# luchsonice/3dod

Measured on AMD Instinct MI355X. Metric: images/sec Cube R-CNN DLA34-FPN train step, higher is better.
Workload: dtype fp32; 1 GPU; Cube R-CNN DLA34+FPN train step (fwd+loss+bwd+allreduce+SGD), 4 img/GPU 512x512, Base_Omni3D.yaml semantics (BASELINE configs[3] per-GPU shard); global_batch=4, parallelism=dp1, weight_gradient_reduce=pixel splits stored and added in a fixed order (CR_DETERMINISTIC=1), valid=True

## Files before the change

3dod_amd/_lib.py:

```python
import ctypes
import os
import threading

import torch

_HERE = os.path.dirname(os.path.abspath(__file__))
LIB_PATH = os.path.join(_HERE, "lib", "libcr3dod.so")

c_void_p, c_int, c_int64, c_float = ctypes.c_void_p, ctypes.c_int, ctypes.c_int64, ctypes.c_float
P = c_void_p

SIGNATURES = {
    "cr_ctx_create": [c_int, P, ctypes.POINTER(P)],
    "cr_ctx_destroy": [P],
    "cr_ctx_set_stream": [P, P],
    "cr_abi_version": [],
    "cr_cuboid_corners": [P, P, P, c_int64, P],
    "cr_cubes_project_score": [P, P, c_int64, c_int64, P, c_int, c_float, c_float, P, P, P, P,
                               P, P, P, P, P, P, P, P, P],
    "cr_cubes_project_score_fast": [P, P, c_int64, c_int64, P, c_int, c_float, c_float, P, P, P, P,
                                    P, P, P, P, P, P, P, P, P, P],
    "cr_propose": [P, P, c_int64, P, c_int, c_int, P, P, P, c_int64, P, c_int, P, P, P, P, P],
    "cr_ransac_plane": [P, P, c_int64, P, c_int64, c_float, P, P, P],
    "cr_ransac_plane_batched": [P, P, P, c_int, c_int64, P, c_int64, c_float, P, P, P],
# ... 18 lines not shown
    "cr_rpn_unpack": [P, P, P, c_int, c_int, c_int, c_int, P, P, P],
    "cr_rpn_pack_grad": [P, P, P, P, P, c_int, c_int, c_int, c_int],
    "cr_topk_blocks": [c_int64, c_int],
    "cr_topk": [P, P, c_int, c_int64, c_int, P, P, P],
    "cr_multi_seg": [P, P, c_int, c_int64, c_int],
    "cr_loss_guard": [P, P, c_int, c_float, P, P, P, c_int, c_float, c_float, P],
    "cr_step_counters": [P, P, P, P],
    "cr_weights_split3": [P, P, P, P, c_int, c_int64],
    "cr_conv2d_bwd_weight": [P, P, P, P, c_int, c_int, c_int, c_int, c_int, c_int, c_int, c_int, c_int, c_int],
    "cr_conv2d_bwd_weight_bias": [P, P, P, P, P, c_int, c_int, c_int, c_int, c_int, c_int, c_int, c_int, c_int, c_int],
    "cr_cast_f32_to_bf16": [P, P, P, c_int64],
    "cr_weight_transpose": [P, P, P, c_int, c_int, c_int, c_int],
    "cr_colsum_accum": [P, P, c_int, c_int64, c_int, P, P],
    "cr_bn_fwd": [P, P, P, c_int, P, P, P, P, c_int64, c_int, c_int, c_float, c_float, P, P, P, c_int],
    "cr_bn_bwd": [P, P, P, P, P, P, P, P, P, P, P, c_int64, c_int, c_int, c_int],
    "cr_bn_frozen_unfold": [P, P, P, P, P, P, P, c_float, P, c_int, P, P, c_int, c_int],
    "cr_pool2x_fwd": [P, P, P, c_int, c_int, c_int, c_int, c_int, c_int],
    "cr_pool2x_bwd": [P, P, P, P, c_int, c_int, c_int, c_int, c_int, c_int, P],
    "cr_upsample2x_add": [P, P, P, P, c_int, c_int, c_int, c_int, c_int],
    "cr_sum2x2": [P, P, P, c_int, c_int, c_int, c_int, c_int],
    "cr_preprocess": [P, P, P, c_int, c_int, c_int, P, P, c_int],
    "cr_roi_align_fwd": [P, P, P, P, P, c_int, c_int, P, c_int64, c_int, c_int, P, c_int],
    "cr_roi_align_bwd": [P, P, P, P, P, c_int, c_int, P, c_int64, c_int, c_int, P, c_int],
    "cr_conv2d_fwd_group": [P, c_int, P, P, P, P, P, P, c_int, c_int, c_int, c_int, P, P, c_int, c_int],
    "cr_wino_filter": [P, P, P, c_int, c_int, c_int],
    "cr_gemm_batched_f32": [P, P, P, P, c_int, c_int, c_int, c_int, c_int64, c_int64, c_int64],
    "cr_wino_input": [P, c_int, P, P, P, P, c_int, P, c_int64],
    "cr_wino_output": [P, c_int, P, P, P, P, P, c_int, c_int64, P, c_int, P],
    "cr_wino_dy": [P, c_int, P, P, P, P, c_int, P, c_int64, P],
    "cr_wino_filter_grad": [P, P, P, c_int, c_int, P, P],
    "cr_wgrad_batched_f32": [P, P, P, P, c_int, c_int, c_int, c_int, c_int64, c_int64, c_int64],
    "cr_conv2d_bwd_data_group": [P, c_int, P, P, P, P, P, P, c_int, c_int, c_int, c_int, c_int, P],
    "cr_conv2d_bwd_weight_group": [P, c_int, P, P, P, P, P, P, P, c_int, c_int, c_int, c_int, c_int],
    "cr_roi_align_bwd_set": [P, P, P, P, P, c_int, c_int, c_int, P, c_int64, c_int, c_int, P, c_int],
    "cr_nms_grouped": [P, P, P, c_int, c_int, c_float, P, P],
    "cr_cube_loss_fwd": [P, P, c_int64, c_int, c_int, c_int, c_int, P, P],
    "cr_cube_loss_bwd": [P, P, c_int64, c_int, c_int, c_int, c_int, P, P, P, P, P, P],
    "cr_rpn_decode_select": [P, P, P, P, P, c_int, c_int, c_int, P, c_float, P, c_float, P, P, P],
    "cr_box_match": [P, P, c_int, P, P, c_int, c_int, c_int, P, P, P, P],
    "cr_rpn_label": [P, P, P, P, P, P, P, c_int, c_int, c_int, c_float, c_float, P, c_float, P, P, P, P],
    "cr_rpn_scatter": [P, P, P, c_int, P, P, c_int, c_int, P, c_float, c_int, c_int, P],
    "cr_rpn_loss": [P, P, P, P, P, P, P, c_int, c_int, c_int, P, P, P, P, P],
    "cr_roi_label": [P, P, P, P, P, P, P, c_int, c_int, c_int, c_int, c_float, c_float, c_float, P, P, P],
    "cr_roi_compact": [P, P, P, c_int, P, P, c_int, c_int, P, P, P, c_int, c_int, P, P, P, P, P],
    "cr_box_loss": [P, P, P, P, P, P, P, P, c_int, c_int, c_int, c_int, P, c_float, P, P, P, P, P],
    "cr_det_scores": [P, P, c_int, P, c_int, P, P, c_int, c_int, c_int, c_int, c_float, P, P],
    "cr_det_gather": [P, P, P, P, c_int, P, P, c_int, c_int, c_int, c_int, c_int, P, c_float, P, P, P, P],
    "cr_nms_grouped_cls": [P, P, P, P, c_int, c_int, c_float, P, P],
    "cr_det_pick": [P, P, P, P, P, P, P, P, P, c_int, c_int, c_int, c_int, c_int, c_int, P, P, P, P, P, P],
    "cr_weak_loss_fwd": [P, P, P, P, P, P, P, P, P, c_int, c_int, c_int, c_int, c_int, c_int, P, P, P, P, P],
    "cr_weak_loss_reduce": [P, P, P, P, P, c_int, c_int, P, P, P, c_int, c_int, c_int, c_int, c_int, c_int, P, P, P, P, P, P, P, P,
                            P, P, P],
    "cr_weak_loss_bwd": [P, P, P, P, P, P, P, P, P, c_int, c_int, c_int, c_int, c_int, c_int, P, P, P, P, P, P, P, P, P, P, P, P],
    "cr_cube_select": [P, P, c_int, P, c_int, P, P, P, c_int, c_int, c_int, c_int, P, P, P, P, P, P, P, c_int, c_int, P, P, P],
    "cr_cube_select_bwd": [P, P, c_int, P, c_int, c_int, c_int, P, P, P, P, P, P, P, P, P, c_int, c_int, P, P, P],
    "cr_cube_reduce": [P, P, P, P, P, c_int, c_int, P, P, P],
    "cr_cube_reduce_bwd": [P, P, P, P, c_int, c_int, P, P, P, P],
    "cr_cube_select_norm": [P, P, c_int, P, c_int, c_int, c_int, P, c_int, c_int, P, P, P, P],
    "cr_cube_nondis_fwd": [P, P, P, c_int64, c_int, c_int, c_int, c_int, P, P],
    "cr_cube_nondis_bwd": [P, P, P, c_int64, c_int, c_int, c_int, c_int, P, P, P, P, P, P, P],
    "cr_cube_select_bwd_zraw": [P, c_int, P, c_int, c_int, c_int, P, P, P, P, c_int, P, P],
    "cr_weights_prepare": [P, P, P, P, P, P, c_int, c_int],
    "cr_fc_weight_prepare": [P, P, P, c_int, c_int, c_int, c_int],
    "cr_fc_grad_accum": [P, P, P, c_int, c_int, c_int, c_int],
    "cr_linear_fwd": [P, P, P, P, P, c_int, c_int, c_int, c_int, c_int, c_int, P],
    "cr_linear_bwd_data": [P, P, P, P, c_int, c_int, c_int, c_int, P],
# ... 104 lines not shown
```

3dod_amd/csrc/conv.hip:

```cpp
#include "cr_common.h"
#include "cr_elem.h"
#include <stdlib.h>
#include <type_traits>

typedef __bf16 bf16x8 __attribute__((ext_vector_type(8)));
typedef __bf16 bf16x4 __attribute__((ext_vector_type(4)));
typedef short s16x4 __attribute__((ext_vector_type(4)));
typedef float f32x4 __attribute__((ext_vector_type(4)));

#define CONV_T 256

struct ConvP {
    const void* x;
    const void* w;
    void* y;
    const void* res;
    const float* bias;
    float* stats;
    int N, Hin, Win, Cin, Hout, Wout, Cout;
    int stride, pad, Kdim, M, cshift, relu;
    unsigned x_bytes, w_bytes;
    int f32;
    float* part;
    int ksplit, kstages;
// ... 1717 lines not shown
            for (int j = 0; j < TJ; ++j) {
                const int kk = q0 + noff + j * 16 + li;
#pragma unroll
                for (int e = 0; e < 4; ++e) {
                    const int ch = c0 + moff + i * 16 + 4 * g + e;
                    if (kk < p.Kdim && ch < p.Cout) atomicAdd(&p.dw[(size_t)ch * p.Kdim + kk], acc[i][j][e]);
                }
            }
    } else {
        float* tile = reinterpret_cast<float*>(smem);
#pragma unroll
        for (int gg = 0; gg < KG; ++gg) {
            if (grp == gg) {
#pragma unroll
                for (int i = 0; i < TI; ++i)
#pragma unroll
                    for (int j = 0; j < TJ; ++j)
#pragma unroll
                        for (int e = 0; e < 4; ++e) {
                            float* d = &tile[(moff + i * 16 + 4 * g + e) * TNP + noff + j * 16 + li];
                            if (gg == 0) *d = acc[i][j][e]; else *d += acc[i][j][e];
                        }
            }
            __syncthreads();
        }
        for (int idx = threadIdx.x; idx < TM * TN; idx += CONV_T * KG) {
            const int chl = idx / TN, kl = idx - chl * TN;
            const int ch = c0 + chl, kk = q0 + kl;
            if (kk < p.Kdim && ch < p.Cout) atomicAdd(&p.dw[(size_t)ch * p.Kdim + kk], tile[chl * TNP + kl]);
        }
    }
}

template <int TM, int KS>
__device__ __forceinline__ void conv_wgrad_f32_body(const WgP& p, const int blk_id, const int blk_count) {
    constexpr int TN = 128, KU = 2, PS = 16;
    constexpr int WM = (TM == 128) ? 2 : 1, WN = 4 / WM;
    constexpr int WTM = TM / WM, WTN = TN / WN;
    constexpr int TI = WTM / 16, TJ = WTN / 16;
    constexpr int PP = ((TM + 16) % 32 == 16) ? TM + 16 : TM + 32, PQ = TN + 16;
    constexpr int CPR = TM / 4;
    constexpr int NP = (PS * CPR + CONV_T - 1) / CONV_T;
    __shared__ __attribute__((aligned(16))) float smem[KU * PS * (PP + PQ)];
    float* sP = smem;
    float* sQ = smem + KU * PS * PP;
    const float* __restrict__ xg = reinterpret_cast<const float*>(p.x);
    (void)xg;

    const int tid = threadIdx.x, lane = tid & 63, wave = tid >> 6;
    const int bid = xcd_swizzle(blk_id, blk_count);
    const int bx = bid % p.tm, by = (bid / p.tm) % p.tn, bz = bid / (p.tm * p.tn);
    const int c0 = bx * TM, q0 = by * TN;
    const int step0 = bz * p.steps_per_split;
    const int nsteps_total = (p.M + PS - 1) / PS;
    const int step1 = min(step0 + p.steps_per_split, nsteps_total);
    if (step0 >= step1) return;

    const int qc = tid & 31;
    const int qk = q0 + qc * 4;
    int qr = 0, qs = 0, qch = qk;
    const bool qvalid = qk < p.Kdim;
    if (KS > 1) {
        const int tap = qk >> p.cshift;
        qch = qk & (p.Cin - 1);
        qr = tap / KS;
        qs = tap - qr * KS;
    }
    int pn[2], pho[2], pwo[2];
    {
        const int hw = p.Hout * p.Wout;
#pragma unroll
        for (int i = 0; i < 2; ++i) {
            const int m = step0 * PS + (tid >> 5) + 8 * i;
            pn[i] = m / hw;
            const int rem = m - pn[i] * hw;
            pho[i] = rem / p.Wout;
// ... 241 lines not shown
    for (int j = 0; j < NCH; ++j) {
        const int f = ((j + (int)blockIdx.x) % NCH) * 256 + tid;
        if (f < NW) {
            const int co = f / (TAPS * CIN), k = f - co * (TAPS * CIN);
            const int i = (k >> 4) * 256 + co * 16 + (k & 15);
            const float v = (sRed[i] + sRed[NT * 256 + i]) + (sRed[2 * NT * 256 + i] + sRed[3 * NT * 256 + i]);
            if (p.slab) p.slab[(size_t)blockIdx.x * p.slab_stride + f] = v;
            else atomicAdd(&p.dw[f], v);
        }
    }
    if (p.dbias != nullptr) {
#pragma unroll
        for (int off = 16; off < 64; off <<= 1) bsum += __shfl_xor(bsum, off, 64);
        if (lane < 16) atomicAdd(&p.dbias[lane], bsum);
    }
}

static int try_launch_wgrad_patch_f32(cr_ctx* ctx, WgP& p, int ks) {
    const bool shape_ok = p.Cout == 16 && p.stride == 1 && p.pad == ks / 2 && (p.Hout & 15) == 0 && (p.Wout & 15) == 0 &&
                          p.Hin == p.Hout && p.Win == p.Wout && ((ks == 3 && p.Cin == 16) || (ks == 7 && p.Cin == 4));
    if (!shape_ok) return NOT_TAKEN;
    const int tiles_x = p.Wout / 16, tiles_per_img = tiles_x * (p.Hout / 16), tiles_total = tiles_per_img * p.N;
    const dim3 grid((unsigned)std::min(tiles_total, 256 * PATCH_BLOCKS_PER_CU));
    size_t ws_off = 0;
    if (deterministic_on() && p.dbias) return NOT_TAKEN;
    const bool slabs = wgrad_use_slabs(ctx, p, (int)grid.x, &ws_off);
    if (ks == 3) hipLaunchKernelGGL((k_conv_wgrad_patch_f32<3, 16>), grid, dim3(256), 0, ctx->stream, p, tiles_x, tiles_per_img, tiles_total);
    else hipLaunchKernelGGL((k_conv_wgrad_patch_f32<7, 4>), grid, dim3(256), 0, ctx->stream, p, tiles_x, tiles_per_img, tiles_total);
    if (slabs) wgrad_reduce_slabs(ctx, p, (int)grid.x);
    CR_LAUNCH_CHECK();
    return CR_OK;
}

template <int KS>
static int launch_wgrad_f32_ks(cr_ctx* ctx, WgP& p) {
    constexpr int PS = 16;
    const int nsteps = (p.M + PS - 1) / PS;
    const int tn = (int)cr_cdiv(p.Kdim, 128);
    int TM = p.Cout >= 128 ? 128 : (p.Cout >= 64 ? 64 : (p.Cout >= 32 ? 32 : 16));
    if (TM == 128 && ((p.Cout == 128 && p.M <= 16384) || (p.Cout == 256 && p.M <= 4096))) TM = 64;
    if (TM == 128 && KS == 1 && p.Cout >= 1024) TM = 64;
    const int tm = (int)cr_cdiv(p.Cout, TM);
    const int tiles = tm * tn;
    const int max_splits = nsteps / 8 > 1 ? nsteps / 8 : 1;
    int splits = 768 / tiles;
    if (tiles > 768 && nsteps >= 32) splits = 2;
    if (splits > max_splits) splits = max_splits;
    if (splits > nsteps) splits = nsteps;
    if (splits < 1) splits = 1;
    p.steps_per_split = (nsteps + splits - 1) / splits;
    p.steps_per_split = (p.steps_per_split + 1) & ~1;
    splits = (nsteps + p.steps_per_split - 1) / p.steps_per_split;
    dim3 grid(tm * tn * splits);
    p.tm = tm; p.tn = tn;
    size_t ws_off = 0;
    const bool slabs = wgrad_use_slabs(ctx, p, splits, &ws_off);
    if (TM == 128) hipLaunchKernelGGL((k_conv_wgrad_f32<128, KS>), grid, dim3(CONV_T), 0, ctx->stream, p);
    else if (TM == 64) hipLaunchKernelGGL((k_conv_wgrad_f32<64, KS>), grid, dim3(CONV_T), 0, ctx->stream, p);
    else if (TM == 32) hipLaunchKernelGGL((k_conv_wgrad_f32<32, KS>), grid, dim3(CONV_T), 0, ctx->stream, p);
    else hipLaunchKernelGGL((k_conv_wgrad_f32<16, KS>), grid, dim3(CONV_T), 0, ctx->stream, p);
    if (slabs) wgrad_reduce_slabs(ctx, p, splits);
    CR_LAUNCH_CHECK();
    return CR_OK;
}

template <int TM, int KS>
__global__ __launch_bounds__(CONV_T * 2) void k_conv_wgrad_s3(WgP p) {
    constexpr int TN = 128;
    constexpr int WM = (TM == 128) ? 2 : 1, WN = 4 / WM;
    constexpr int WTM = TM / WM, WTN = TN / WN;
    constexpr int TI = WTM / 16, TJ = WTN / 16;
    constexpr int PP = TM == 128 ? 144 : TM + 8, PQ = TN + 16;
    auto rotQ = [](int row, int col) { return (col + (((row >> 3) & 1) << 6)) & 127; };
    auto rotP = [&](int row, int col) { return TM == 128 ? rotQ(row, col) : col; };
    constexpr int CPR = TM / 8;
    constexpr int NP = (32 * CPR + CONV_T - 1) / CONV_T;
    constexpr int PE = 32 * PP, QE = 32 * PQ;
    constexpr int GE = 3 * (PE + QE);
    constexpr int TNP = TN + 4;
    static_assert(TM * TNP * 4 <= 2 * GE * 2, "reduction tile must fit in the operand images");
    __shared__ __attribute__((aligned(16))) u16 smem[2 * GE];
    const int grp = (int)(threadIdx.x >> 8);
    u16* sP = smem + grp * GE;
    u16* sQ = sP + 3 * PE;

    const int tid = threadIdx.x & (CONV_T - 1), lane = tid & 63, wave = tid >> 6;
    const int bid = xcd_swizzle(blockIdx.x, gridDim.x);
// ... 558 lines not shown
    const int tm = Cout / 128, tn = (int)cr_cdiv((int64_t)ks * ks * Cin, 128), tiles = tm * tn;
    int splits_all = 768 / tiles > 1 ? 768 / tiles : 1;
    int sps = (int)cr_cdiv(steps_all, splits_all);
    if (sps < 8) sps = 8;
    sps = (sps + 1) & ~1;
    for (int i = 0; i < n; ++i) {
        CR_CHECK_ARG(dys[i] && xs[i] && dws[i], "cr_conv2d_bwd_weight_group: NULL tensor %d", i);
        int rc = conv_common_checks("cr_conv2d_bwd_weight_group", Ns[i], Hs[i], Ws[i], Cin, Cout, ks, 1, pad, act_f32);
        if (rc) return rc;
        const int H = Hs[i], W = Ws[i], Ho = H + 2 * pad - ks + 1, Wo = W + 2 * pad - ks + 1;
        WgP& p = g.p[i];
        p = make_wgrad_params(dys[i], xs[i], dws[i], Ns[i], H, W, Cin, Ho, Wo, Cout, ks, 1, pad, act_f32);
        p.dbias = dbiases ? dbiases[i] : nullptr;
        const int nsteps = (p.M + PS - 1) / PS;
        p.steps_per_split = sps;
        p.tm = tm; p.tn = tn;
        counts[i] = tiles * (int)cr_cdiv(nsteps, sps);
    }
    size_t ws_off = 0;
    bool slabs = deterministic_on();
    for (int i = 0; i < n && slabs; ++i) slabs = wgrad_use_slabs(ctx, g.p[i], counts[i] / tiles, &ws_off);
    if (!slabs)
        for (int i = 0; i < n; ++i) { g.p[i].slab = nullptr; g.p[i].bslab = nullptr; g.p[i].slab_stride = 0; }
    const int total = group_starts(n, counts, g.start);
    for (int i = 0; i < n; ++i) g.count[i] = counts[i];
    for (int i = n; i < CR_MAX_GROUP; ++i) { g.start[i] = total; g.count[i] = 0; }
    const dim3 grid((unsigned)total), block(CONV_T);
    if (ks == 1) hipLaunchKernelGGL(k_conv_wgrad_f32_grp<1>, grid, block, 0, ctx->stream, g);
    else hipLaunchKernelGGL(k_conv_wgrad_f32_grp<3>, grid, block, 0, ctx->stream, g);
    if (slabs)
        for (int i = 0; i < n; ++i) wgrad_reduce_slabs(ctx, g.p[i], counts[i] / tiles);
    CR_LAUNCH_CHECK();
    return CR_OK;
}

__global__ void k_cast_f32_bf16(const float* __restrict__ src, u16* __restrict__ dst, int64_t n) {
    const int64_t i = ((int64_t)blockIdx.x * blockDim.x + threadIdx.x) * 4;
    if (i + 3 < n) {
        const float4 v = *reinterpret_cast<const float4*>(src + i);
        uint2 pk;
        pk.x = (unsigned)f2bf(v.x) | ((unsigned)f2bf(v.y) << 16);
        pk.y = (unsigned)f2bf(v.z) | ((unsigned)f2bf(v.w) << 16);
        *reinterpret_cast<uint2*>(dst + i) = pk;
    } else {
        for (int64_t j = i; j < n; ++j) dst[j] = f2bf(src[j]);
    }
}

template <typename T>
__global__ __launch_bounds__(256) void k_fold_bn(const float* __restrict__ w, const float* __restrict__ gamma,
                                                 const float* __restrict__ beta, const float* __restrict__ mean,
                                                 const float* __restrict__ var, float eps, T* __restrict__ wf,
                                                 float* __restrict__ bias, int Cout, int K) {
    const int co = blockIdx.x;
    const float s = gamma[co] * rsqrtf(var[co] + eps);
    if (threadIdx.x == 0) bias[co] = beta[co] - mean[co] * s;
    const float* wr = w + (size_t)co * K;
    T* o = wf + (size_t)co * K;
    for (int i = threadIdx.x; i < K; i += 256) {
        if constexpr (sizeof(T) == 2) o[i] = f2bf(wr[i] * s); else o[i] = wr[i] * s;
    }
}

extern "C" int cr_fold_bn(cr_ctx* ctx, const float* w, const float* gamma, const float* beta, const float* mean,
                          const float* var, float eps, void* wf, float* bias, int Cout, int K, int act_f32) {
    CR_CHECK_ARG(ctx && w && gamma && beta && mean && var && wf && bias && Cout > 0 && K > 0, "cr_fold_bn: bad args");
// ... 968 lines not shown
```

3dod_amd/cubercnn/modeling/graphed.py:

```python
import contextlib
import gc

import torch
import torch.nn as nn

from ... import hipops as ops


@contextlib.contextmanager
def capture_guard():
    was = gc.isenabled()
    gc.collect()
    _empty_graveyard()
    gc.disable()
    keep, prev = [], ops._PLAN_KEEP[0]
    ops._PLAN_KEEP[0] = keep
    try:
        yield keep
    finally:
        ops._PLAN_KEEP[0] = prev
        if was:
            gc.enable()
        _empty_graveyard()

# ... 101 lines not shown
        bu = getattr(model.backbone, "bottom_up", None)
        lower = [getattr(bu, n, None) for n in ("base_layer", "level0", "level1", "level2", "level3", "level4")]
        self.split = bool(split_backward) and bu is not None and all(m is not None for m in lower) and hasattr(bu, "level5")
        cut = {}
        self.trigger = torch.zeros((), device=dev, requires_grad=True)
        pg = model.proposal_generator
        self.feat_names = None

        def dense():
            x = ops.preprocess(self.static_img, model.pixel_mean_list, model.pixel_std_list)
            feats = model.backbone(x)
            ys = pg.rpn_head.forward_raw([feats[f] for f in pg.in_features])
            self.feat_names = list(feats.keys())
            self.n_levels = len(ys)
            return tuple(feats.values()) + tuple(ys)

        mods = [model.backbone, pg.rpn_head]

        def leaves():
            ps = [p for m in mods for p in m.parameters() if p.requires_grad]
            for p in ps:
                assert ops.grad_sink(p) is not None, "build the optimizer (FlatSGD) before capturing graphs"
            return ps

        def lower_ids():
            return {id(p) for m in lower for p in m.parameters()}

        def segment_params(first):
            low = lower_ids()
            return [p for m in mods for p in m.parameters() if p.requires_grad and ((id(p) not in low) == first)]
        self.segment_params = segment_params

        def run_backward(outs, grads):
            ps = leaves()
            keep_o, keep_g = [], []
            for o, g in zip(outs, grads):
                slot = getattr(o, "_cr_slot", None)
                if slot is not None and ops._SLOTS_ON[0]:
                    ops._slot_put(slot, g)
                else:
                    keep_o.append(o); keep_g.append(g)
            if not self.split:
                res = torch.autograd.grad(keep_o, ps, keep_g, allow_unused=True)
                for p, g in zip(ps, res):
                    if g is not None:
                        ops.grad_sink(p).add_(g)
                return None
            low = lower_ids()
            ps1 = [p for p in ps if id(p) not in low]
            res = torch.autograd.grad(keep_o, ps1 + [cut["x"]], keep_g, allow_unused=True, retain_graph=True)
            for p, g in zip(ps1, res[:-1]):
                if g is not None:
                    ops.grad_sink(p).add_(g)
            assert res[-1] is not None, "two-segment backward: no gradient reaches the trunk"
            return res[-1]

        def run_backward2(gx):
            low = lower_ids()
            ps2 = [p for p in leaves() if id(p) in low]
            res = torch.autograd.grad([cut["x"]], ps2, [gx], allow_unused=True)
            for p, g in zip(ps2, res):
                if g is not None:
                    ops.grad_sink(p).add_(g)

        bn_state = [(m, m.running_mean.clone(), m.running_var.clone(), m.num_batches_tracked.clone())
                    for mod in mods for m in mod.modules()
                    if isinstance(m, nn.BatchNorm2d) and m.running_mean is not None]
        self.bank = next((getattr(p, "_cr_bank")[0] for mod in mods for p in mod.parameters() if hasattr(p, "_cr_bank")), None)
        s = torch.cuda.Stream(device=dev)
        s.wait_stream(torch.cuda.current_stream(dev))
        hook = bu.level4.register_forward_hook(lambda m, i, o: cut.__setitem__("x", o)) if self.split else None
        with torch.cuda.stream(s), _fresh_leaves(mods):
            for _ in range(warmup):
                outs = dense()
                gx = run_backward(outs, tuple(torch.zeros_like(o) for o in outs))
                if self.split:
                    run_backward2(gx)
            del outs
        torch.cuda.current_stream(dev).wait_stream(s)
        torch.cuda.synchronize(dev)

        ops.bump_weight_epoch()
        with capture_guard() as self._keep, _fresh_leaves(mods):
            self.fwd_graph = torch.cuda.CUDAGraph()
            with torch.cuda.graph(self.fwd_graph):
                self.static_outs = dense()
            self.static_grads = tuple(torch.zeros_like(o) for o in self.static_outs)
            self.bwd_graph = torch.cuda.CUDAGraph()
            with torch.cuda.graph(self.bwd_graph, pool=self.fwd_graph.pool()):
                gx = run_backward(self.static_outs, self.static_grads)
# ... 77 lines not shown
```

3dod_amd/cubercnn/solver/build.py:

```python
from typing import Any, Dict, List

import torch
import torch.distributed as dist

from ... import hipops as ops
from ..modeling.graphed import GraphOwner as _GraphOwner

NORM_TYPES = (torch.nn.BatchNorm1d, torch.nn.BatchNorm2d, torch.nn.BatchNorm3d, torch.nn.SyncBatchNorm,
              torch.nn.GroupNorm, torch.nn.InstanceNorm1d, torch.nn.InstanceNorm2d, torch.nn.InstanceNorm3d,
              torch.nn.LayerNorm, torch.nn.LocalResponseNorm)
NO_DECAY_KEYS = ('priors_dims_per_cat', 'priors_z_scales', 'priors_z_stats')


def freeze_bn(network):
    for _, module in network.named_modules():
        if isinstance(module, torch.nn.BatchNorm2d):
            module.eval()
            module.track_running_stats = False


def _param_groups(cfg, model):
    memo, groups = set(), []
    for module in model.modules():
        for key, value in module.named_parameters(recurse=False):
            if not value.requires_grad or value in memo:
                continue
            memo.add(value)
            lr, wd = cfg.SOLVER.BASE_LR, cfg.SOLVER.WEIGHT_DECAY
            if isinstance(module, NORM_TYPES) and cfg.SOLVER.WEIGHT_DECAY_NORM is not None:
                wd = cfg.SOLVER.WEIGHT_DECAY_NORM
            elif key == "bias":
                if cfg.SOLVER.BIAS_LR_FACTOR is not None:
                    lr = cfg.SOLVER.BASE_LR * cfg.SOLVER.BIAS_LR_FACTOR
                if cfg.SOLVER.WEIGHT_DECAY_BIAS is not None:
                    wd = cfg.SOLVER.WEIGHT_DECAY_BIAS
            if key in NO_DECAY_KEYS:
                wd = 0.0
            groups.append((value, float(lr), float(wd)))
# ... 282 lines not shown
        with torch.cuda.stream(self.comm_stream):
            for a, b in self.early_ranges:
                dist.all_reduce(self.opt.flat_g[a:b])
        self._early_done = True

    def __call__(self, data):
        opt, world = self.opt, self.world
        loss_dict = self.model(data)
        keys = sorted(loss_dict.keys())
        vals = torch.stack([loss_dict[k].float() for k in keys])
        losses = vals.sum()
        red = vals.detach().clone()
        if world > 1:
            if self.comm_stream is not None:
                self.comm_stream.wait_stream(torch.cuda.current_stream())
                with torch.cuda.stream(self.comm_stream):
                    dist.all_reduce(red)
                red.record_stream(self.comm_stream)
            else:
                dist.all_reduce(red)
        opt.zero_grad()
        g = getattr(self.model, "_graphed", None)
        if g is not None and self.comm_stream is not None and g.pre_bwd is None:
            g.pre_bwd = self._early_allreduce
        if g is not None and self.comm_stream is not None and getattr(g, "bwd_graph2", None) is not None and g.mid_bwd is None:
            early = set(self.early_ranges)
            mid = [r for r in param_ranges(g.segment_params(True), opt) if r not in early]
            self.mid_ranges = [(x, min(x + self._bucket, b)) for a, b in mid for x in range(a, b, self._bucket)]
            self._mid_whole = mid
            self.late_after_mid = complement_ranges(sorted(self.early_ranges + mid), opt.flat_g.numel(), self._bucket)
            self.__dict__.pop("_rest_cache", None)
            g.mid_bwd = self._mid_allreduce
        self._early_done = self._mid_done = False
        losses.backward()
        opt.collect_grads()
        if self.comm_stream is not None and (world > 1 or self.force_comm):
            self.comm_stream.wait_stream(torch.cuda.current_stream())
            with torch.cuda.stream(self.comm_stream):
                for a, b in self._rest_ranges():
                    dist.all_reduce(opt.flat_g[a:b])
            torch.cuda.current_stream().wait_stream(self.comm_stream)
        elif world > 1:
            for a, b in self.buckets:
                dist.all_reduce(opt.flat_g[a:b])
        losses_reduced = torch.empty((), dtype=torch.float32, device=red.device)
        ops.loss_guard(red, 1.0 / world, red, losses_reduced, self.recent_loss, self.stabilize, self.TOLERANCE, self.GAMMA,
                       self.flag)
        if self.stabilize:
            ops.nonfinite_flag(opt.flat_g, self.flag)
        opt.step(skip_flag=self.flag, grad_scale=1.0 / world)
        ops.step_counters(self.flag, self.iterations_explode, self.iterations_success)
        self.last = {"keys": keys, "values": red, "total": losses_reduced, "skipped": self.flag}
        return self.last

    def report(self):
        d = {k: float(v) for k, v in zip(self.last["keys"], self.last["values"].tolist())}
        d["total_loss"] = float(self.last["total"])
        d["iterations_explode"] = float(self.iterations_explode)
        d["iterations_success"] = float(self.iterations_success)
        return d


class GraphedTrainStep(_GraphOwner):
    G_PAD = 32
    TOLERANCE, GAMMA = TrainStep.TOLERANCE, TrainStep.GAMMA

    def __init__(self, cfg, model, optimizer, sample_data, world_size=1, bucket_mb=32, warmup=2):
# ... 137 lines not shown
```

3dod_amd/hipops.py:

```python
import ctypes
import os

import torch

from . import _lib

bf16 = torch.bfloat16
f32 = torch.float32
STAT_REPL = 32

_PRECISIONS = {"fp32": (f32, 1), "f32": (f32, 1), "float32": (f32, 1), "fp32x3": (f32, 2), "bf16": (bf16, 0),
               "bfloat16": (bf16, 0)}
_ACT = [_PRECISIONS[os.environ.get("CR_PRECISION", "fp32").lower()]]


def set_precision(name):
    prev = precision()
    _ACT[0] = _PRECISIONS[str(name).lower()]
    return prev


def precision():
    return {0: "bf16", 1: "fp32", 2: "fp32x3"}[_ACT[0][1]]


def act_dtype():
    return _ACT[0][0]


def _af(t):
    if t.dtype == f32:
        return _ACT[0][1] if _ACT[0][0] == f32 else 1
# ... 191 lines not shown
            return None, 0
        slot = _GradSlot(f"tensor {tuple(x.shape)}")
        try:
            x._cr_slot = slot
        except Exception:
            return None, 0
    slot.n_reg += 1
    return slot, slot.n_reg


def _slot_put(slot, g):
    if slot.done:
        raise RuntimeError("gradient slot: a contribution arrived after the accumulating convolution's backward had run "
                           "(set CR_GRAD_SLOTS=0 to fall back to autograd's adds)")
    slot.buf = g if slot.buf is None else slot.buf + g
    slot.n_arr += 1


def _slot_fold(slot):
    buf, slot.buf = slot.buf, None
    return buf


def _slot_take(slot):
    slot.done = True
    buf, slot.buf = slot.buf, None
    return buf


def grad_sink(t):
    return getattr(t, "_cr_grad", None)


def conv_bwd_weight_raw(dy, x, k, stride, pad, sink=None, bias_acc=None):
    N, H, W, Cin = x.shape
    Cout = dy.shape[3]
    af = _af(x)
    assert dy.dtype == x.dtype
    if bias_acc is not None:
        dw = sink if sink is not None else torch.empty((Cout, Cin, k, k), dtype=f32, device=x.device).contiguous(
            memory_format=torch.channels_last)
        _lib.call("cr_conv2d_bwd_weight_bias", dy, x, dw, bias_acc, N, H, W, Cin, Cout, k, stride, pad, int(sink is not None),
                  af)
        return None if sink is not None else dw
    if sink is not None:
        _lib.call("cr_conv2d_bwd_weight", dy, x, sink, N, H, W, Cin, Cout, k, stride, pad, 1, af)
        return None
    dw = torch.empty((Cout, Cin, k, k), dtype=f32, device=x.device).contiguous(memory_format=torch.channels_last)
    _lib.call("cr_conv2d_bwd_weight", dy, x, dw, N, H, W, Cin, Cout, k, stride, pad, 0, af)
    return dw


class _ConvBN(torch.autograd.Function):
    @staticmethod
    def forward(ctx, x, weight, gamma, beta, residual, running_mean, running_var, stride, pad, relu, eps, momentum,
                training, slots=((None, 0), (None, 0))):
        ctx.slots = slots
        Cout, Cin, k, _ = weight.shape
        dev = x.device
        af = _af(x)
        if training:
            wb, _ = prepared_weights(weight, x.requires_grad, x.dtype)
            _STATS_EPOCH[0] += 1
            N_, H_, W_, _ = x.shape
            M = N_ * ((H_ + 2 * pad - k) // stride + 1) * ((W_ + 2 * pad - k) // stride + 1)
            nparts = (M + 63) // 64
            stats = torch.empty((nparts, 2, Cout), dtype=f32, device=dev)
            y_raw = conv_fwd_raw(x, wb, Cout, k, stride, pad, stats=stats)
            out = torch.empty_like(y_raw)
            mi = torch.empty((2, Cout), dtype=f32, device=dev)
            _lib.call("cr_bn_fwd", y_raw, stats, nparts, gamma.detach(), beta.detach(), residual, out, M, Cout, int(relu),
# ... 1773 lines not shown
```

include/cr3dod.h:

```cpp
#ifndef CR3DOD_H
#define CR3DOD_H

#include <stdint.h>

#ifdef __cplusplus
extern "C" {
#endif

typedef struct cr_ctx cr_ctx;

#define CR_OK 0
#define CR_EINVAL (-22)
#define CR_ENOMEM (-12)
#define CR_EHIP (-5)
#define CR_ERANGE (-34)

int cr_ctx_create(int device, void* hip_stream, cr_ctx** out);
int cr_ctx_destroy(cr_ctx* ctx);
int cr_ctx_set_stream(cr_ctx* ctx, void* hip_stream);
const char* cr_last_error(void);
int cr_abi_version(void);


int cr_cuboid_corners(cr_ctx* ctx, const float* box6, const float* R, int64_t n, float* verts);
// ... 76 lines not shown
int cr_topk(cr_ctx* ctx, const float* x, int rows, int64_t n, int k, void* ws, float* vals, int64_t* idx);
int cr_loss_guard(cr_ctx* ctx, const float* vals, int n, float scale, float* red, float* total, float* recent,
                  int stabilize, float tolerance, float gamma, int* flag);
int cr_step_counters(cr_ctx* ctx, const int* flag, float* explode, float* success);
int cr_multi_seg(cr_ctx* ctx, const void* descs_dev, int ndesc, int64_t total, int accumulate);
int cr_relu_bwd(cr_ctx* ctx, const void* y, const void* dy, void* g, int64_t n, int act_f32);
int cr_fold_bn(cr_ctx* ctx, const float* w, const float* gamma, const float* beta, const float* mean, const float* var,
               float eps, void* wf, float* bias, int Cout, int K, int act_f32);

int cr_conv2d_bwd_weight_bias(cr_ctx* ctx, const void* dy, const void* x, float* dw, float* dbias, int N, int H, int W,
                              int Cin, int Cout, int ks, int stride, int pad, int accumulate, int act_f32);
int cr_wino_filter(cr_ctx* ctx, const float* w_krsc, float* U, int O, int C, int backward);
int cr_gemm_batched_f32(cr_ctx* ctx, const float* x, const float* w, float* y, int R, int K, int O, int batches,
                        int64_t stride_x, int64_t stride_w, int64_t stride_y);
int cr_wino_input(cr_ctx* ctx, int n, const float* const* xs, const int* Ns, const int* Hs, const int* Ws, int C,
                  float* V, int64_t T);
int cr_wino_output(cr_ctx* ctx, int n, const float* M, float* const* ys, const int* Ns, const int* Hs, const int* Ws,
                   int O, int64_t T, const float* bias, int relu, const float* const* accs);
int cr_wino_dy(cr_ctx* ctx, int n, const float* const* dys, const int* Ns, const int* Hs, const int* Ws, int O,
               float* dM, int64_t T, float* db_part);
int cr_wino_filter_grad(cr_ctx* ctx, const float* dU, float* dw, int O, int C, const float* db_part, float* db);
int cr_wgrad_batched_f32(cr_ctx* ctx, const float* dy, const float* x, float* dw, int R, int K, int O, int batches,
                         int64_t stride_dy, int64_t stride_x, int64_t stride_dw);

int cr_conv2d_fwd_group(cr_ctx* ctx, int n, const void* const* xs, const void* const* ws, void* const* ys, const int* Ns,
                        const int* Hs, const int* Ws, int Cin, int Cout, int ks, int pad, const float* const* biases,
                        const void* const* residuals, int relu, int act_f32);
int cr_conv2d_bwd_data_group(cr_ctx* ctx, int n, const void* const* dys, const void* const* wts, void* const* dxs,
                             const int* Ns, const int* Hs, const int* Ws, int Cin, int Cout, int ks, int pad, int act_f32,
                             const void* const* accumulates);
int cr_conv2d_bwd_weight_group(cr_ctx* ctx, int n, const void* const* dys, const void* const* xs, float* const* dws,
                               float* const* dbiases, const int* Ns, const int* Hs, const int* Ws, int Cin, int Cout, int ks,
                               int pad, int act_f32);
int cr_cast_f32_to_bf16(cr_ctx* ctx, const float* src, void* dst, int64_t n);
int cr_colsum_accum(cr_ctx* ctx, const void* x, int is_f32, int64_t M, int C, float* ws, float* out);
int cr_weight_transpose(cr_ctx* ctx, const float* w, void* wt, int Cout, int ks, int Cin, int act_f32);

int cr_bn_fwd(cr_ctx* ctx, const void* x, const float* stats, int nparts, const float* gamma, const float* beta,
              const void* residual, void* y, int64_t M, int C, int relu, float eps, float momentum,
              float* mean_invstd, float* running_mean, float* running_var, int act_f32);
int cr_bn_bwd(cr_ctx* ctx, const void* dy, const void* out, const void* x, const float* mean_invstd,
              const float* gamma, float* sums, void* dx, void* dres, float* dgamma, float* dbeta, int64_t M,
              int C, int relu, int act_f32);
int cr_bn_frozen_unfold(cr_ctx* ctx, const float* dwf, const float* sg, const float* w, const float* gamma,
                        const float* mean, const float* var, float eps, float* dw, int accumulate, float* dgamma,
                        float* dbeta, int Cout, int K);

int cr_pool2x_fwd(cr_ctx* ctx, const void* x, void* y, int N, int H, int W, int C, int window, int act_f32);
int cr_pool2x_bwd(cr_ctx* ctx, const void* x, const void* dy, void* dx, int N, int H, int W, int C, int window, int act_f32,
                  const void* accumulate);
int cr_upsample2x_add(cr_ctx* ctx, const void* lat, const void* top, void* y, int N, int H, int W, int C, int act_f32);
int cr_sum2x2(cr_ctx* ctx, const void* dy, void* dtop, int N, int H, int W, int C, int act_f32);
int cr_preprocess(cr_ctx* ctx, const unsigned char* img, void* y, int N, int H, int W, const float* mean3,
                  const float* std3, int act_f32);

int cr_roi_align_fwd(cr_ctx* ctx, const void* const* feats, const int* Hs, const int* Ws, const float* scales,
                     int nlev, int C, const float* rois, int64_t R, int PH, int PW, void* out, int act_f32);
int cr_roi_align_bwd(cr_ctx* ctx, float* const* grads, const int* Hs, const int* Ws, const float* scales,
                     int nlev, int C, const float* rois, int64_t R, int PH, int PW, const void* dout, int act_f32);
int cr_roi_align_bwd_set(cr_ctx* ctx, float* const* grads, const int* Hs, const int* Ws, const float* scales,
                         int nlev, int C, int N, const float* rois, int64_t R, int PH, int PW, const void* dout,
                         int act_f32);
int cr_nms_grouped(cr_ctx* ctx, const float* boxes, const int* counts, int G, int maxn, float thresh,
                   void* mask_ws, unsigned char* keep);

int cr_cube_loss_fwd(cr_ctx* ctx, const float* const* inputs, int64_t n, int allocentric, int chamfer_pose,
// ... 130 lines not shown
```

Baseline: 271.1 images/s.

## Defer conv weight-gradient kernels during backward and batch them into one multi-shape launch

```diff
diff --git a/3dod_amd/_lib.py b/3dod_amd/_lib.py
--- a/3dod_amd/_lib.py
+++ b/3dod_amd/_lib.py
@@ -74,6 +74,7 @@
     "cr_wgrad_batched_f32": [P, P, P, P, c_int, c_int, c_int, c_int, c_int64, c_int64, c_int64],
     "cr_conv2d_bwd_data_group": [P, c_int, P, P, P, P, P, P, c_int, c_int, c_int, c_int, c_int, P],
     "cr_conv2d_bwd_weight_group": [P, c_int, P, P, P, P, P, P, P, c_int, c_int, c_int, c_int, c_int],
+    "cr_conv2d_bwd_weight_multi": [P, c_int, P, P, P, P, P, P, P, P, P, P, P, P, c_int],
     "cr_roi_align_bwd_set": [P, P, P, P, P, c_int, c_int, c_int, P, c_int64, c_int, c_int, P, c_int],
     "cr_nms_grouped": [P, P, P, c_int, c_int, c_float, P, P],
     "cr_cube_loss_fwd": [P, P, c_int64, c_int, c_int, c_int, c_int, P, P],
diff --git a/3dod_amd/csrc/conv.hip b/3dod_amd/csrc/conv.hip
--- a/3dod_amd/csrc/conv.hip
+++ b/3dod_amd/csrc/conv.hip
@@ -1773,7 +1773,12 @@
     }
 }
 
-template <int TM, int KS>
+__device__ __forceinline__ float* wgrad_f32_lds_pool() {
+    __shared__ __attribute__((aligned(16))) float pool[2 * 16 * (144 + 144)];
+    return pool;
+}
+
+template <int TM, int KS, bool POOLED = false>
 __device__ __forceinline__ void conv_wgrad_f32_body(const WgP& p, const int blk_id, const int blk_count) {
     constexpr int TN = 128, KU = 2, PS = 16;
     constexpr int WM = (TM == 128) ? 2 : 1, WN = 4 / WM;
@@ -1782,7 +1787,14 @@
     constexpr int PP = ((TM + 16) % 32 == 16) ? TM + 16 : TM + 32, PQ = TN + 16;
     constexpr int CPR = TM / 4;
     constexpr int NP = (PS * CPR + CONV_T - 1) / CONV_T;
-    __shared__ __attribute__((aligned(16))) float smem[KU * PS * (PP + PQ)];
+    float* smem;
+    if constexpr (POOLED) {
+        static_assert(KU * PS * (PP + PQ) <= 2 * 16 * (144 + 144), "wgrad_f32_lds_pool too small");
+        smem = wgrad_f32_lds_pool();
+    } else {
+        __shared__ __attribute__((aligned(16))) float own[KU * PS * (PP + PQ)];
+        smem = own;
+    }
     float* sP = smem;
     float* sQ = smem + KU * PS * PP;
     const float* __restrict__ xg = reinterpret_cast<const float*>(p.x);
@@ -2090,8 +2102,7 @@
     return CR_OK;
 }
 
-template <int KS>
-static int launch_wgrad_f32_ks(cr_ctx* ctx, WgP& p) {
+static int plan_wgrad_f32(WgP& p, int KS, int* splits_out) {
     constexpr int PS = 16;
     const int nsteps = (p.M + PS - 1) / PS;
     const int tn = (int)cr_cdiv(p.Kdim, 128);
@@ -2109,8 +2120,16 @@
     p.steps_per_split = (nsteps + splits - 1) / splits;
     p.steps_per_split = (p.steps_per_split + 1) & ~1;
     splits = (nsteps + p.steps_per_split - 1) / p.steps_per_split;
-    dim3 grid(tm * tn * splits);
     p.tm = tm; p.tn = tn;
+    *splits_out = splits;
+    return TM;
+}
+
+template <int KS>
+static int launch_wgrad_f32_ks(cr_ctx* ctx, WgP& p) {
+    int splits;
+    const int TM = plan_wgrad_f32(p, KS, &splits);
+    dim3 grid(p.tm * p.tn * splits);
     size_t ws_off = 0;
     const bool slabs = wgrad_use_slabs(ctx, p, splits, &ws_off);
     if (TM == 128) hipLaunchKernelGGL((k_conv_wgrad_f32<128, KS>), grid, dim3(CONV_T), 0, ctx->stream, p);
@@ -2735,6 +2754,115 @@
         for (int i = 0; i < n; ++i) wgrad_reduce_slabs(ctx, g.p[i], counts[i] / tiles);
     CR_LAUNCH_CHECK();
     return CR_OK;
+}
+
+struct WgMulti { WgP p[CR_MAX_GROUP]; int start[CR_MAX_GROUP], count[CR_MAX_GROUP], cls[CR_MAX_GROUP]; int n; };
+
+__global__ __launch_bounds__(CONV_T) void k_conv_wgrad_f32_multi(WgMulti g) {
+    int i = 0;
+    while (i + 1 < g.n && (int)blockIdx.x >= g.start[i + 1]) ++i;
+    const int blk = (int)blockIdx.x - g.start[i];
+    if (blk >= g.count[i]) return;
+    switch (g.cls[i]) {
+    case 0: conv_wgrad_f32_body<64, 1, true>(g.p[i], blk, g.count[i]); break;
+    case 1: conv_wgrad_f32_body<64, 3, true>(g.p[i], blk, g.count[i]); break;
+    case 2: conv_wgrad_f32_body<128, 1, true>(g.p[i], blk, g.count[i]); break;
+    default: conv_wgrad_f32_body<128, 3, true>(g.p[i], blk, g.count[i]); break;
+    }
+}
+
+static void plan_wgrad_f32_group(WgP* ps, int n, int* TMs, int* splits) {
+    constexpr int PS = 16;
+    int nsteps[CR_MAX_GROUP], tiles[CR_MAX_GROUP];
+    int64_t work = 0;
+    for (int i = 0; i < n; ++i) {
+        WgP& p = ps[i];
+        TMs[i] = p.Cout >= 128 ? 128 : 64;
+        p.tm = (int)cr_cdiv(p.Cout, TMs[i]); p.tn = (int)cr_cdiv(p.Kdim, 128);
+        tiles[i] = p.tm * p.tn;
+        nsteps[i] = (p.M + PS - 1) / PS;
+        work += (int64_t)tiles[i] * nsteps[i] * (TMs[i] / 64);
+    }
+    int64_t per_block = cr_cdiv(work, 768);
+    for (int it = 0; it < 6; ++it) {
+        int64_t total = 0;
+        for (int i = 0; i < n; ++i) {
+            int sps = (int)cr_cdiv(per_block, TMs[i] / 64);
+            if (sps < 8) sps = 8;
+            sps = (sps + 1) & ~1;
+            ps[i].steps_per_split = sps;
+            splits[i] = (int)cr_cdiv(nsteps[i], sps);
+            total += ((int64_t)tiles[i] * splits[i] + 7) & ~(int64_t)7;
+        }
+        if (total <= 768) break;
+        per_block = cr_cdiv(per_block * total, 768) + 1;
+    }
+}
+
+static int launch_wgrad_f32_multi(cr_ctx* ctx, WgMulti& g, const int* splits) {
+    int counts[CR_MAX_GROUP];
+    for (int i = 0; i < g.n; ++i) counts[i] = g.p[i].tm * g.p[i].tn * splits[i];
+    const int total = group_starts(g.n, counts, g.start);
+    for (int i = 0; i < g.n; ++i) g.count[i] = counts[i];
+    for (int i = g.n; i < CR_MAX_GROUP; ++i) { g.start[i] = total; g.count[i] = 0; g.cls[i] = 0; }
+    hipLaunchKernelGGL(k_conv_wgrad_f32_multi, dim3((unsigned)total), dim3(CONV_T), 0, ctx->stream, g);
+    for (int i = 0; i < g.n; ++i)
+        if (g.p[i].slab) wgrad_reduce_slabs(ctx, g.p[i], splits[i]);
+    CR_LAUNCH_CHECK();
+    g.n = 0;
+    return CR_OK;
+}
+
+extern "C" int cr_conv2d_bwd_weight_multi(cr_ctx* ctx, int n, const void* const* dys, const void* const* xs, float* const* dws,
+                                          float* const* dbiases, const int* Ns, const int* Hs, const int* Ws, const int* Cins,
+                                          const int* Couts, const int* kss, const int* strides, const int* pads, int act_f32) {
+    CR_CHECK_ARG(ctx && dys && xs && dws && Ns && Hs && Ws && Cins && Couts && kss && strides && pads,
+                 "cr_conv2d_bwd_weight_multi: NULL pointer");
+    CR_CHECK_ARG(n >= 1, "cr_conv2d_bwd_weight_multi: n >= 1");
+    const bool det = deterministic_on() && ctx->ws;
+    WgMulti g;
+    g.n = 0;
+    int splits[CR_MAX_GROUP], TMs[CR_MAX_GROUP];
+    size_t ws_off = 0;
+    int rc;
+    auto flush = [&]() -> int {
+        ws_off = 0;
+        if (g.n == 0) return CR_OK;
+        if (!det) plan_wgrad_f32_group(g.p, g.n, TMs, splits);
+        for (int i = 0; i < g.n; ++i) g.cls[i] = (TMs[i] == 128 ? 2 : 0) + (g.p[i].Kdim == 9 * g.p[i].Cin ? 1 : 0);
+        return launch_wgrad_f32_multi(ctx, g, splits);
+    };
+    for (int i = 0; i < n; ++i) {
+        float* const dbias = dbiases ? dbiases[i] : nullptr;
+        const int N = Ns[i], H = Hs[i], W = Ws[i], Cin = Cins[i], Cout = Couts[i], ks = kss[i], stride = strides[i], pad = pads[i];
+        bool grouped = act_f32 == 1 && dys[i] && xs[i] && dws[i] && (ks == 1 || ks == 3) && Cout >= 64;
+        WgP p{};
+        if (grouped) {
+            if ((rc = conv_common_checks("cr_conv2d_bwd_weight_multi", N, H, W, Cin, Cout, ks, stride, pad, act_f32))) return rc;
+            const int Ho = (H + 2 * pad - ks) / stride + 1, Wo = (W + 2 * pad - ks) / stride + 1;
+            p = make_wgrad_params(dys[i], xs[i], dws[i], N, H, W, Cin, Ho, Wo, Cout, ks, stride, pad, act_f32);
+            p.dbias = dbias;
+            if (det) {
+                int sp;
+                const int TM = plan_wgrad_f32(p, ks, &sp);
+                grouped = TM >= 64;
+                if (grouped && !wgrad_use_slabs(ctx, p, sp, &ws_off)) {
+                    if ((rc = flush())) return rc;
+                    grouped = wgrad_use_slabs(ctx, p, sp, &ws_off);
+                }
+                if (grouped) { TMs[g.n] = TM; splits[g.n] = sp; }
+            }
+        }
+        if (!grouped) {
+            if ((rc = flush())) return rc;
+            if ((rc = conv2d_bwd_weight_impl(ctx, dys[i], xs[i], dws[i], dbias, N, H, W, Cin, Cout, ks, stride, pad, 1, act_f32)))
+                return rc;
+            continue;
+        }
+        g.p[g.n++] = p;
+        if (g.n == CR_MAX_GROUP && (rc = flush())) return rc;
+    }
+    return flush();
 }
 
 __global__ void k_cast_f32_bf16(const float* __restrict__ src, u16* __restrict__ dst, int64_t n) {
diff --git a/3dod_amd/cubercnn/modeling/graphed.py b/3dod_amd/cubercnn/modeling/graphed.py
--- a/3dod_amd/cubercnn/modeling/graphed.py
+++ b/3dod_amd/cubercnn/modeling/graphed.py
@@ -157,6 +157,14 @@
         self.segment_params = segment_params
 
         def run_backward(outs, grads):
+            with ops.deferred_wgrad():
+                return _run_backward(outs, grads)
+
+        def run_backward2(gx):
+            with ops.deferred_wgrad():
+                _run_backward2(gx)
+
+        def _run_backward(outs, grads):
             ps = leaves()
             keep_o, keep_g = [], []
             for o, g in zip(outs, grads):
@@ -180,7 +188,7 @@
             assert res[-1] is not None, "two-segment backward: no gradient reaches the trunk"
             return res[-1]
 
-        def run_backward2(gx):
+        def _run_backward2(gx):
             low = lower_ids()
             ps2 = [p for p in leaves() if id(p) in low]
             res = torch.autograd.grad([cut["x"]], ps2, [gx], allow_unused=True)
diff --git a/3dod_amd/cubercnn/solver/build.py b/3dod_amd/cubercnn/solver/build.py
--- a/3dod_amd/cubercnn/solver/build.py
+++ b/3dod_amd/cubercnn/solver/build.py
@@ -4,6 +4,7 @@
 import torch.distributed as dist
 
 from ... import hipops as ops
+from ...hipops import deferred_wgrad
 from ..modeling.graphed import GraphOwner as _GraphOwner
 
 NORM_TYPES = (torch.nn.BatchNorm1d, torch.nn.BatchNorm2d, torch.nn.BatchNorm3d, torch.nn.SyncBatchNorm,
@@ -352,7 +353,8 @@
             self.__dict__.pop("_rest_cache", None)
             g.mid_bwd = self._mid_allreduce
         self._early_done = self._mid_done = False
-        losses.backward()
+        with deferred_wgrad():
+            losses.backward()
         opt.collect_grads()
         if self.comm_stream is not None and (world > 1 or self.force_comm):
             self.comm_stream.wait_stream(torch.cuda.current_stream())
diff --git a/3dod_amd/hipops.py b/3dod_amd/hipops.py
--- a/3dod_amd/hipops.py
+++ b/3dod_amd/hipops.py
@@ -1,3 +1,4 @@
+import contextlib
 import ctypes
 import os
 
@@ -255,11 +256,53 @@
     return getattr(t, "_cr_grad", None)
 
 
+WGRAD_GROUP = 8
+_WGRAD_DEPTH = [0]
+_WGRAD_PENDING = []
+
+
+def wgrad_pending():
+    return len(_WGRAD_PENDING)
+
+
+def conv_bwd_weight_multi_raw(items):
+    cast = lambda a: ctypes.cast(a, ctypes.c_void_p)
+    xs = [it[1] for it in items]
+    _lib.call("cr_conv2d_bwd_weight_multi", len(items), cast(_ptr_table([it[0] for it in items])), cast(_ptr_table(xs)),
+              cast(_ptr_table([it[2] for it in items])), cast(_ptr_table([it[3] for it in items])),
+              cast(_int_table([x.shape[0] for x in xs])), cast(_int_table([x.shape[1] for x in xs])),
+              cast(_int_table([x.shape[2] for x in xs])), cast(_int_table([x.shape[3] for x in xs])),
+              cast(_int_table([it[0].shape[3] for it in items])), cast(_int_table([it[4] for it in items])),
+              cast(_int_table([it[5] for it in items])), cast(_int_table([it[6] for it in items])), 1, device=xs[0].device)
+
+
+def wgrad_flush():
+    if _WGRAD_PENDING:
+        items = list(_WGRAD_PENDING)
+        del _WGRAD_PENDING[:]
+        conv_bwd_weight_multi_raw(items)
+
+
+@contextlib.contextmanager
+def deferred_wgrad():
+    _WGRAD_DEPTH[0] += 1
+    try:
+        yield
+    finally:
+        _WGRAD_DEPTH[0] -= 1
+        wgrad_flush()
+
+
 def conv_bwd_weight_raw(dy, x, k, stride, pad, sink=None, bias_acc=None):
     N, H, W, Cin = x.shape
     Cout = dy.shape[3]
     af = _af(x)
     assert dy.dtype == x.dtype
+    if sink is not None and af == 1 and _WGRAD_DEPTH[0] > 0:
+        _WGRAD_PENDING.append((dy, x, sink, bias_acc, k, stride, pad))
+        if len(_WGRAD_PENDING) >= WGRAD_GROUP:
+            wgrad_flush()
+        return None
     if bias_acc is not None:
         dw = sink if sink is not None else torch.empty((Cout, Cin, k, k), dtype=f32, device=x.device).contiguous(
             memory_format=torch.channels_last)
diff --git a/include/cr3dod.h b/include/cr3dod.h
--- a/include/cr3dod.h
+++ b/include/cr3dod.h
@@ -132,6 +132,9 @@
 int cr_conv2d_bwd_weight_group(cr_ctx* ctx, int n, const void* const* dys, const void* const* xs, float* const* dws,
                                float* const* dbiases, const int* Ns, const int* Hs, const int* Ws, int Cin, int Cout, int ks,
                                int pad, int act_f32);
+int cr_conv2d_bwd_weight_multi(cr_ctx* ctx, int n, const void* const* dys, const void* const* xs, float* const* dws,
+                               float* const* dbiases, const int* Ns, const int* Hs, const int* Ws, const int* Cins,
+                               const int* Couts, const int* kss, const int* strides, const int* pads, int act_f32);
 int cr_cast_f32_to_bf16(cr_ctx* ctx, const float* src, void* dst, int64_t n);
 int cr_colsum_accum(cr_ctx* ctx, const void* x, int is_f32, int64_t M, int C, float* ws, float* out);
 int cr_weight_transpose(cr_ctx* ctx, const float* w, void* wt, int Cout, int ks, int Cin, int act_f32);
```

After: 280.2 images/s, median of 6. 3.3% higher.
